# RobinWitch/SynTalker

Measured on AMD Instinct MI355X. Metric: denoising-steps/sec (128-frame clips), higher is better.
Workload: dtype bf16; 1 GPU; diffusion_rvqvae_128.yaml sampling: DDPM p_sample_loop steps (1000-step schedule), 1024 clips/GPU x (1536,1,32) latents, MDM denoiser 8x512, random-init; clips_per_gpu=1024, global_clips=1024, parallelism=clip-sharded x1, no collective, primed_steps=0, m_tile=auto

## Files before the change

### syntalker_amd/csrc/syn_kernels.hip

```cpp
#include <hip/hip_runtime.h>
#include <stdint.h>
#include <stdio.h>
#include <stdlib.h>
#include <string.h>

#include "syn_hip.h"

typedef __attribute__((ext_vector_type(8))) __bf16 bf16x8;
typedef __attribute__((ext_vector_type(4))) __bf16 bf16x4;
typedef __attribute__((ext_vector_type(4))) float f32x4;

#define MFMA16(a, b, c) __builtin_amdgcn_mfma_f32_16x16x32_bf16((a), (b), (c), 0, 0, 0)

namespace {

constexpr int kThreads = 512;
constexpr int kKT = 64;
constexpr int kNT = 512;

enum Epi { EPI_PLAIN = 0, EPI_IN = 1, EPI_QKV = 2, EPI_RESID = 3, EPI_GELU = 4, EPI_OUT = 5 };

struct GArgs {
    const __bf16* X; long x_chunk_stride; int ldx; int x_rows;
    const uint4* W; int K; int M;
// ... 1473 lines not shown
        if (hipGetDevice(&dev) != hipSuccess || dev < 0 || dev >= kMaxDevices) return true;
        if (done[dev]) return false;
        done[dev] = true;
        return true;
    }
};

void n128_setup() {
    static OncePerDevice once;
    if (once.first()) {
        allow_lds(k_gemm_n128, kN128Lds);
        allow_lds(k_gemm_pair<16, 2>, kN128Lds);
        allow_lds(k_gemm_and_pack<16, 2>, kN128Lds);
        allow_lds(k_gemm_quad_all, kN128Lds);
    }
}

struct StackInstance {
    int rows, tp;
    bool edit;
    void (*kernel)(SArgs);
    OncePerDevice once;
    int lds() const { return rows * 2048 + 4096; }
};
StackInstance* stack_instance(int rows, int tp, bool edit) {
    static StackInstance table[] = {
        {64, 0, false, k_stack<64>},          {32, 0, false, k_stack<32>},
        {64, 0, true,  k_stack<64, 0, true>}, {32, 0, true,  k_stack<32, 0, true>}, {32, 2, true, k_stack<32, 2, true>}, {32, 4, true, k_stack<32, 4, true>},
        {32, 2, false, k_stack<32, 2>},       {32, 4, false, k_stack<32, 4>},       {64, 2, false, k_stack<64, 2>},
    };
    for (StackInstance& i : table)
        if (i.rows == rows && i.tp == tp && i.edit == edit) return &i;
    return nullptr;
}

int launch_stack(const SArgs& a, int mt, hipStream_t s) {
    const bool edit = a.out.keep != nullptr;
    dim3 grid((a.M + mt - 1) / mt), block(kThreads);
    if (a.tp > 1) {
        if (!(mt == 32 || (mt == 64 && a.tp == 2)) || !a.sync || !a.xch) return fail_msg("stack: the tile-split mode needs 32-row tiles (or 64-row tiles split in two), ws_sync and ws_xch");
        grid.x = lat::kGroups * a.tp * ((a.tp_tiles + lat::kGroups - 1) / lat::kGroups);
        if (grid.x > 256) return fail_msg("stack: the tensor-parallel mode needs all its workgroups resident (<= 256)");
        if (edit && mt != 32) return fail_msg("stack: an edit takes split tiles of 32 rows only");
        if (a.tp != 2 && a.tp != 4) return fail_msg("stack: tile split over 2 or 4 workgroups only");
    }
    StackInstance* const k = stack_instance(mt, a.tp > 1 ? a.tp : 0, edit);
    if (!k) return fail_msg("stack: m_tile must be 32 or 64");
    if (k->once.first()) allow_lds(k->kernel, k->lds());
    hipLaunchKernelGGL(k->kernel, grid, block, k->lds(), s, a);
    return launched("k_stack launch");
}

}

#include "syn_stack_train.inc"
#include "syn_seq.inc"
#include "syn_cond.inc"
#include "syn_wavenc.inc"
#include "syn_train.inc"
#include "syn_conv_train.inc"
#include "syn_glue.inc"
#include "syn_rvq.inc"
#include "syn_rvq_train.inc"
#include "syn_pose.inc"
#include "syn_tmr.inc"
#include "syn_bert.inc"
#include "syn_skel.inc"
#include "syn_t2m.inc"
#include "syn_plms.inc"
#include "syn_bpd.inc"
#include "syn_guide.inc"
#include "syn_joints.inc"
#include "syn_mesh.inc"

namespace {

int launch_latency(const lat::LArgs& a, hipStream_t s) {
    static OncePerDevice once;
    if (once.first()) { allow_lds(lat::k_lat, lat::kLds); }
    hipLaunchKernelGGL(lat::k_lat, dim3(lat::kGroups * lat::kP), dim3(kThreads), lat::kLds, s, a);
    return launched("k_lat launch");
}

template <bool G, int NZ>
void launch_seq_as(const seq::QArgs& a, const dim3 grid, hipStream_t s) {
    static OncePerDevice once;
    if (once.first()) { allow_lds(seq::k_seq<G, NZ>, seq::kLds); }
    hipLaunchKernelGGL((seq::k_seq<G, NZ>), grid, dim3(seq::kThreads), seq::kLds, s, a);
}

int launch_seq(const seq::QArgs& a, hipStream_t s) {
    const dim3 grid(a.n_wg > 0 ? a.n_wg : seq_grid(a.R, a.V));
    const int nz = a.noise ? 1 : a.rng ? 2 : 0;
    if (a.V == 1) {
        if (nz == 2) launch_seq_as<false, 2>(a, grid, s); else if (nz == 1) launch_seq_as<false, 1>(a, grid, s); else launch_seq_as<false, 0>(a, grid, s);
    } else {
        if (nz == 2) launch_seq_as<true, 2>(a, grid, s); else if (nz == 1) launch_seq_as<true, 1>(a, grid, s); else launch_seq_as<true, 0>(a, grid, s);
    }
    return launched("k_seq launch");
}

}

extern "C" {

int syn_version(void) { return SYN_ABI_VERSION; }

void syn_debug_timing(long long* attn_buf, long long* mlp_buf) { g_dbg_attn = attn_buf; g_dbg_mlp = mlp_buf; }
const char* syn_last_error(void) { return g_err; }

int syn_pack_weight(const float* w, int32_t n, int32_t k, void* out_packed, void* stream) {
    if (!w || !out_packed || n % 16 || k % 32) return fail_msg("syn_pack_weight: need n%16==0, k%32==0, non-null pointers");
    const int total = (n / 16) * (k / 32) * 64;
    hipLaunchKernelGGL(k_pack, dim3((total + 255) / 256), dim3(256), 0, (hipStream_t)stream, w, n, k, (uint4*)out_packed);
    return launched("k_pack launch");
}

int syn_pack_weights(const syn_pack_job* jobs_dev, int32_t n_jobs, int64_t max_fragments, void* stream) {
    static_assert(sizeof(syn_pack_job) == sizeof(PackJob), "syn_pack_job is PackJob");
    if (!jobs_dev || n_jobs <= 0 || max_fragments <= 0) return fail_msg("syn_pack_weights: bad arguments");
    hipLaunchKernelGGL(k_pack_many, dim3((unsigned)((max_fragments * 64 + 255) / 256), n_jobs), dim3(256), 0, (hipStream_t)stream,
                       reinterpret_cast<const PackJob*>(jobs_dev));
    return launched("k_pack_many launch");
}

int syn_pack_weight_t(const void* s_kn, int32_t is_bf16, int32_t n, int32_t k, void* out_packed, void* stream) {
    if (!s_kn || !out_packed || n % 16 || k % 32) return fail_msg("syn_pack_weight_t: need n%16==0, k%32==0, non-null pointers");
    const int total = (n / 16) * (k / 32) * 64;
    if (is_bf16)
        hipLaunchKernelGGL(k_pack_t<__bf16>, dim3((total + 255) / 256), dim3(256), 0, (hipStream_t)stream, (const __bf16*)s_kn, n, k,
                           (uint4*)out_packed);
    else
        hipLaunchKernelGGL(k_pack_t<float>, dim3((total + 255) / 256), dim3(256), 0, (hipStream_t)stream, (const float*)s_kn, n, k,
                           (uint4*)out_packed);
    return launched("k_pack_t launch");
}

int syn_to_token_major(const float* x_bct, int32_t n_clips, float* out_f32, void* out_bf16, void* stream) {
    if (!x_bct || n_clips <= 0) return fail_msg("syn_to_token_major: bad arguments");
    hipLaunchKernelGGL(k_to_token_major, dim3(n_clips, SYN_C / 64), dim3(256), 0, (hipStream_t)stream, x_bct, out_f32,
                       (__bf16*)out_bf16);
    return launched("k_to_token_major launch");
}

int32_t syn_prefers_fragment_order(int32_t n_clips, int32_t n_variants) { return prefers_fragment_order(n_clips, n_variants, device_cus()); }

int syn_x_to_fragment(const float* x_bct, int32_t n_clips, float* out_f32, void* out_bf16, void* stream) {
    if (!x_bct || n_clips <= 0) return fail_msg("syn_x_to_fragment: bad arguments");
    hipLaunchKernelGGL(seq::k_x_to_fragment, dim3(n_clips, SYN_C / 32), dim3(256), 0, (hipStream_t)stream, x_bct, out_f32, (uint4*)out_bf16);
    return launched("k_x_to_fragment launch");
}

int syn_x_from_fragment(const float* x_frag, int32_t n_clips, float* out_bct, void* stream) {
    if (!x_frag || !out_bct || n_clips <= 0) return fail_msg("syn_x_from_fragment: bad arguments");
    hipLaunchKernelGGL(seq::k_x_from_fragment, dim3(n_clips, SYN_C / 32), dim3(256), 0, (hipStream_t)stream, x_frag, out_bct);
    return launched("k_x_from_fragment launch");
}

int syn_from_token_major(const float* x_btc, int32_t n_clips, float* out_bct, void* stream) {
    if (!x_btc || !out_bct || n_clips <= 0) return fail_msg("syn_from_token_major: bad arguments");
    hipLaunchKernelGGL(k_from_token_major, dim3(n_clips, SYN_C / 64), dim3(256), 0, (hipStream_t)stream, x_btc, out_bct);
    return launched("k_from_token_major launch");
}

int syn_axpby_rows(const float* x, const float* y, const float* coef_ab, const int32_t* t_row, int32_t n_clips,
                   int32_t per_clip, float* out, void* stream) {
    if (!x || !y || !coef_ab || !t_row || !out || n_clips <= 0 || per_clip % 4) return fail_msg("syn_axpby_rows: bad arguments");
    const long n4 = (long)n_clips * per_clip / 4;
    hipLaunchKernelGGL(k_axpby_rows, dim3((unsigned)((n4 + 255) / 256)), dim3(256), 0, (hipStream_t)stream, x, y, coef_ab,
                       t_row, n4, per_clip / 4, out);
    return launched("k_axpby_rows launch");
}

int syn_steps_advance(const int32_t* sched, int32_t* counter, int32_t* t_model, int32_t n_t_model, int32_t* t_coef, int32_t n_t_coef,
                      int32_t n_steps, void* stream) {
    if (!sched || !counter || !t_model || !t_coef || n_t_model <= 0 || n_t_coef <= 0 || n_steps <= 0)
        return fail_msg("syn_steps_advance: bad arguments");
    hipLaunchKernelGGL(k_step_advance, dim3(1), dim3(256), 0, (hipStream_t)stream, (const int*)sched, (int*)counter, (int*)t_model,
                       n_t_model, (int*)t_coef, n_t_coef, n_steps);
    return launched("k_step_advance launch");
// ... 452 lines not shown
```

### syntalker_amd/csrc/syn_seq.inc

```
namespace {
namespace seq {

typedef __attribute__((ext_vector_type(16))) float f32x16;
#define MFMA32(a, b, c) __builtin_amdgcn_mfma_f32_32x32x16_bf16((a), (b), (c), 0, 0, 0)

#ifndef SEQ_ABL
#define SEQ_ABL 0
#endif
#ifndef SEQ_ABL2
#define SEQ_ABL2 0
#endif
constexpr int kThreads = 256;
constexpr int kFragBytes = 1024;
#ifndef SEQ_CHUNK
#define SEQ_CHUNK 16
#endif
#ifndef SEQ_WIN
#define SEQ_WIN 4
#endif
#ifndef SEQ_SPREAD
#define SEQ_SPREAD 1
#endif
#ifndef SEQ_SCHED
#define SEQ_SCHED 0
#endif
constexpr int kChunkFrags = SEQ_CHUNK, kChunkBytes = kChunkFrags * kFragBytes;
constexpr int kPerWave = kChunkFrags / 4;
constexpr int kSlots = 80 / kChunkFrags, kLook = kSlots - 1;
constexpr int kRingBytes = kSlots * kChunkBytes;
constexpr int kBiasSet = 2048;
constexpr int kRingBase = 0;
constexpr int kBiasBase = kRingBytes;
constexpr int kSlabBase = kBiasBase + 2 * kBiasSet * 4;
constexpr int kSlabBytes = 4 * 4096;
constexpr int kLds = kSlabBase + 4 * kSlabBytes;
#if SEQ_CHUNK == 16
#define SEQ_WAIT_STEADY "s_waitcnt vmcnt(8)"
#define SEQ_WAIT_FIRST "s_waitcnt vmcnt(12)"
#else
#define SEQ_WAIT_STEADY "s_waitcnt vmcnt(14)"
#define SEQ_WAIT_FIRST "s_waitcnt vmcnt(16)"
#endif

struct QArgs {
    const char* tape; unsigned tape_chunks;
    const float* bias;
    const float* te; const float* rcos; const float* rsin;
    const float* cond; const int* t_model;
    const float* xt;
    const uint4* xb;
    const float* noise;
    const unsigned long long* rng; const float* coef; const int* t_coef;
    float* xn; uint4* xnb; float* x0;
    int R;
    int V;
    const float* cfg_w;
    int cfg_stride;
    int n_steps;
    int tm_stride, tc_stride;
    int wg0, n_wg;
    int dbg_step;
    unsigned skew;
    long long* dbg;
};

__device__ __forceinline__ void dma_frag(const char* src, unsigned lds_dst, unsigned lane16) {
    unsigned keep;
    asm volatile("s_mov_b32 %0, m0\n\t"
                 "s_mov_b32 m0, %2\n\t"
                 "s_nop 0\n\t"
                 "global_load_lds_dwordx4 %1, %3\n\t"
                 "s_mov_b32 m0, %0"
                 : "=&s"(keep) : "v"(lane16), "s"(lds_dst), "s"(src) : "memory");
}

template <int OFF>
__device__ __forceinline__ void dma_frag_at(const char* src, unsigned lds_dst, unsigned lane16) {
    asm volatile("s_mov_b32 m0, %1\n\t"
                 "s_nop 0\n\t"
                 "global_load_lds_dwordx4 %0, %2 offset:%c3"
                 :: "v"(lane16), "s"(lds_dst), "s"(src), "i"(OFF) : "memory");
}

#ifndef SEQ_DMA_POL
#define SEQ_DMA_POL 0
#endif
#if SEQ_DMA_POL == 1
#define SEQ_DMA_POLICY " nt"
#elif SEQ_DMA_POL == 2
#define SEQ_DMA_POLICY " sc1"
#elif SEQ_DMA_POL == 3
#define SEQ_DMA_POLICY " sc0"
#else
#define SEQ_DMA_POLICY ""
#endif
struct Ring {
    const char* tape;
    unsigned voff;
    unsigned dst;
    unsigned wq;
    unsigned voff0;
    unsigned lane16;
    unsigned cur, nxt;
    bf16x8 win[SEQ_WIN];
};
static_assert(SEQ_CHUNK == 16 && kPerWave == 4, "the pinned ring arithmetic below is written for 16-fragment chunks");

template <int OFF>
__device__ __forceinline__ void ring_dma(const Ring& r) {
    asm volatile("s_add_u32 m0, %1, %2\n\t"
                 "s_nop 0\n\t"
                 "global_load_lds_dwordx4 %0, %3 offset:%c4" SEQ_DMA_POLICY
                 :: "v"(r.voff), "s"(r.dst), "s"(r.wq), "s"(r.tape), "i"(OFF) : "memory", "scc");
}
__device__ __forceinline__ void ring_dma_i(const Ring& r, int i) {
    switch (i) {
        case 0: ring_dma<0>(r); break;
        case 1: ring_dma<1024>(r); break;
        case 2: ring_dma<2048>(r); break;
        default: ring_dma<3072>(r); break;
    }
}
__device__ __forceinline__ void ring_advance_dma(Ring& r) {
    const unsigned d = r.dst + kChunkBytes;
    r.dst = d == (unsigned)kRingBytes ? 0u : d;
    r.voff += kChunkBytes;
}
__device__ __forceinline__ void ring_next_base(Ring& r) {
    static_assert(kSlots == 5 && kRingBase == 0, "slot arithmetic");
    unsigned t = r.dst + 2 * kChunkBytes;
    t = t >= (unsigned)kRingBytes ? t - kRingBytes : t;
    r.nxt = r.lane16 + t;
}

__device__ __forceinline__ void bias_issue(const float* bias, const Ring& r, int set) {
    const char* src = reinterpret_cast<const char*>(bias + (size_t)set * kBiasSet) + r.wq / 2;
    const unsigned dst = kBiasBase + (set & 1) * (kBiasSet * 4) + r.wq / 2;
    dma_frag(src, dst, r.lane16);
    dma_frag(src + kFragBytes, dst + kFragBytes, r.lane16);
}

__device__ __forceinline__ void ring_boundary(Ring& r) {
    if (!(SEQ_ABL & 2)) {
        if (!(SEQ_ABL & 64)) asm volatile(SEQ_WAIT_STEADY ::: "memory");
        if (!(SEQ_ABL & 128)) __builtin_amdgcn_s_barrier();
    }
    r.cur = r.nxt;
}

__device__ __forceinline__ bf16x8 take(Ring& r, const char* lds, int& f) {
    if (f == 0) {
        const bf16x8 a = r.win[0];
        if (!(SEQ_ABL & 4)) r.win[0] = *reinterpret_cast<const bf16x8*>(lds + r.nxt + SEQ_WIN * kFragBytes);
        ring_boundary(r);
        __builtin_amdgcn_sched_barrier(0);
        f = 1;
        return a;
    }
    if (!(SEQ_ABL & 1) && (f & 3) == 2) ring_dma_i(r, f >> 2);
    if (f == 6) ring_next_base(r);
    if (f == 15) ring_advance_dma(r);
    const bf16x8 a = r.win[f & (SEQ_WIN - 1)];
    const int g = f + SEQ_WIN;
    if (!(SEQ_ABL & 4))
        r.win[f & (SEQ_WIN - 1)] = *reinterpret_cast<const bf16x8*>(lds + (g < kChunkFrags ? r.cur + g * kFragBytes : r.nxt + (g - kChunkFrags) * kFragBytes));
#if SEQ_SCHED == 0
    __builtin_amdgcn_sched_barrier(0);
#else
    __builtin_amdgcn_sched_group_barrier(0x100, 1, 0);
    __builtin_amdgcn_sched_group_barrier(0x008, 1, 0);
    __builtin_amdgcn_sched_group_barrier(0x002, SEQ_SCHED, 0);
#endif
    f = (f + 1) & (kChunkFrags - 1);
    return a;
}

__device__ __forceinline__ bf16x8 pack8(const f32x16& t, int c) {
    bf16x8 o;
#pragma unroll
    for (int e = 0; e < 8; ++e) o[e] = (__bf16)t[8 * c + e];
    return o;
}

__device__ __forceinline__ f32x16 zero16() {
    f32x16 z;
#pragma unroll
    for (int v = 0; v < 16; ++v) z[v] = 0.f;
    return z;
}

__device__ __forceinline__ f32x16 bias_tile(const char* lds, int set, int off, int tile, int hi) {
    unsigned at = (unsigned)(kBiasBase + (set & 1) * (kBiasSet * 4) + (off + 32 * tile + 4 * hi) * 4);
    asm volatile("" : "+v"(at));
    const float* b = reinterpret_cast<const float*>(lds + at);
    f32x16 o;
#pragma unroll
    for (int q = 0; q < 4; ++q) {
        const f32x4 v = *reinterpret_cast<const f32x4*>(b + 8 * q);
        o[4 * q] = v[0]; o[4 * q + 1] = v[1]; o[4 * q + 2] = v[2]; o[4 * q + 3] = v[3];
    }
    return o;
}

__device__ __forceinline__ f32x16 slab_load(const char* slab, int t) {
    f32x16 o;
#pragma unroll
    for (int q = 0; q < 4; ++q) {
        const f32x4 v = *reinterpret_cast<const f32x4*>(slab + (t * 4 + q) * 1024);
        o[4 * q] = v[0]; o[4 * q + 1] = v[1]; o[4 * q + 2] = v[2]; o[4 * q + 3] = v[3];
    }
    return o;
}
__device__ __forceinline__ void slab_store(char* slab, int t, const f32x16& v) {
#pragma unroll
    for (int q = 0; q < 4; ++q)
        *reinterpret_cast<f32x4*>(slab + (t * 4 + q) * 1024) = f32x4{v[4 * q], v[4 * q + 1], v[4 * q + 2], v[4 * q + 3]};
}

__device__ __forceinline__ float xor32(float v) { return __shfl_xor(v, 32); }

__device__ __forceinline__ float gelu_fast(float x) {
    if (SEQ_ABL2 & 1) return x;
    const float x2 = fminf(x * x, 64.0f);
    float t = fmaf(1.0142633e-3f, x2, -1.0677573e-1f);
    t = fmaf(t, x2, -2.3011213f);
    const float e = __builtin_amdgcn_exp2f(x * t);
    return nopk(x * __builtin_amdgcn_rcpf(1.0f + e));
}

struct NoFill { __device__ __forceinline__ void operator()(int) const {} };

__device__ __forceinline__ void slab_load_half(const char* slab, int t, int half, f32x16& o) {
#pragma unroll
    for (int q = 2 * half; q < 2 * half + 2; ++q) {
        const f32x4 v = *reinterpret_cast<const f32x4*>(slab + (t * 4 + q) * 1024);
        o[4 * q] = v[0]; o[4 * q + 1] = v[1]; o[4 * q + 2] = v[2]; o[4 * q + 3] = v[3];
    }
}
__device__ __forceinline__ void slab_store_quad(char* slab, int t, int q, const f32x16& v) {
    *reinterpret_cast<f32x4*>(slab + (t * 4 + q) * 1024) = f32x4{v[4 * q], v[4 * q + 1], v[4 * q + 2], v[4 * q + 3]};
}

template <int KC, int SPLIT = 0, typename Opnd, typename Fill = NoFill>
__device__ __forceinline__ void wide_of(Ring& r, const char* lds, f32x16 (&h)[12], char* slab, Opnd opnd, Fill fill = Fill()) {
    static_assert(SPLIT >= 0 && SPLIT < KC && (SPLIT == 0 || 12 * SPLIT >= 20), "slab loads must fit in front of their first use");
    constexpr int kLoad0 = SPLIT ? 12 * SPLIT - 12 : 0;
    constexpr int kStore0 = KC > 1 ? 16 * (KC - 1) + 4 : 16 * KC;
    f32x16 s[4];
    int f = 0, n = 0;
    auto mm = [&](f32x16& acc, int kc) {
        acc = MFMA32(take(r, lds, f), opnd(kc), acc);
        if (n >= kLoad0 && n < kLoad0 + 8) slab_load_half(slab, (n - kLoad0) >> 1, (n - kLoad0) & 1, s[(n - kLoad0) >> 1]);
        if (n >= kStore0 && n < kStore0 + 12) {
            const int j = n - kStore0, first = j < 4 ? 2 * j : 4 + j, cnt = j < 4 ? 2 : 1;
#pragma unroll
            for (int w = first; w < first + cnt; ++w) slab_store_quad(slab, w >> 2, w & 3, s[w >> 2]);
        }
        fill(n);
        ++n;
    };
    if constexpr (SPLIT > 0) {
#pragma unroll
        for (int kc = 0; kc < SPLIT; ++kc)
#pragma unroll
            for (int t = 0; t < 12; ++t) mm(h[t], kc);
#pragma unroll
        for (int kc = 0; kc < SPLIT; ++kc)
#pragma unroll
            for (int t = 0; t < 4; ++t) mm(s[t], kc);
    }
#pragma unroll
    for (int kc = SPLIT; kc < KC; ++kc) {
        if (KC > 1 && kc == KC - 1) {
#pragma unroll
            for (int t = 0; t < 4; ++t) mm(s[t], kc);
#pragma unroll
            for (int t = 0; t < 12; ++t) mm(h[t], kc);
        } else {
#pragma unroll
            for (int t = 0; t < 12; ++t) mm(h[t], kc);
#pragma unroll
            for (int t = 0; t < 4; ++t) mm(s[t], kc);
        }
    }
    if constexpr (KC == 1) {
#pragma unroll
        for (int t = 0; t < 4; ++t) slab_store(slab, t, s[t]);
    }
}

template <int KC, typename Fill = NoFill>
__device__ __forceinline__ void wide(Ring& r, const char* lds, f32x16 (&h)[12], char* slab, bf16x8 (&B)[KC], Fill fill = Fill()) {
    wide_of<KC, 0>(r, lds, h, slab, [&](int kc) { return B[kc]; }, fill);
}

template <bool SWAP, typename Fill = NoFill>
__device__ __forceinline__ void pair512(Ring& r, const char* lds, const bf16x8 (&B)[32], f32x16& a0, f32x16& a1, Fill fill = Fill()) {
    int f = 0;
#pragma unroll
    for (int kc = 0; kc < 32; ++kc) {
        const bf16x8 w0 = take(r, lds, f);
        a0 = SWAP ? MFMA32(B[kc], w0, a0) : MFMA32(w0, B[kc], a0);
        const bf16x8 w1 = take(r, lds, f);
        a1 = SWAP ? MFMA32(B[kc], w1, a1) : MFMA32(w1, B[kc], a1);
        fill(kc);
    }
}

typedef float f32x2 __attribute__((ext_vector_type(2)));
__device__ __forceinline__ f32x2 pk_add(f32x2 a, f32x2 b) { return a + b; }
__device__ __forceinline__ f32x2 pk_fma(f32x2 a, f32x2 b, f32x2 c) { return a * b + c; }

__device__ __forceinline__ void norm_to_operands(const f32x16 (&h)[12], const char* slab, bf16x8 (&xn)[32]) {
    if (SEQ_ABL2 & 16) {
#pragma unroll
        for (int i = 0; i < 32; ++i)
#pragma unroll
            for (int e = 0; e < 8; ++e) xn[i][e] = (__bf16)0.01f;
        return;
    }
    f32x2 s2 = {0.f, 0.f}, q2 = {0.f, 0.f};
#pragma unroll
    for (int t = 0; t < 16; ++t) {
        const f32x16 v = t < 12 ? h[t] : slab_load(slab, t - 12);
#pragma unroll
        for (int i = 0; i < 8; ++i) {
            const f32x2 p = {v[2 * i], v[2 * i + 1]};
            s2 = pk_add(s2, p);
            q2 = pk_fma(p, p, q2);
        }
    }
    float s = s2[0] + s2[1], q = q2[0] + q2[1];
    if (SEQ_ABL2 & 2) { s = 1.f; q = 600.f; }
    s += xor32(s); q += xor32(q);
    const float mean = s * (1.0f / 512.0f);
    const float var = fmaxf(q * (1.0f / 512.0f) - mean * mean, 0.f);
    const float rstd = rsqrtf(var + 1e-5f);
    const float nm = -mean * rstd;
    const f32x2 r2 = {rstd, rstd}, n2 = {nm, nm};
#pragma unroll
    for (int t = 0; t < 16; ++t) {
        const f32x16 v = t < 12 ? h[t] : slab_load(slab, t - 12);
#pragma unroll
        for (int c = 0; c < 2; ++c) {
            bf16x8 o;
#pragma unroll
            for (int e = 0; e < 4; ++e) {
                const f32x2 y = pk_fma(f32x2{v[8 * c + 2 * e], v[8 * c + 2 * e + 1]}, r2, n2);
                o[2 * e] = (__bf16)y[0]; o[2 * e + 1] = (__bf16)y[1];
            }
            xn[2 * t + c] = o;
        }
    }
}

using KArgs = const __attribute__((address_space(4))) QArgs;
#define KARGS(name) KArgs* name = reinterpret_cast<KArgs*>(reinterpret_cast<unsigned long long>(__builtin_amdgcn_kernarg_segment_ptr())); asm volatile("" : "+s"(name))

template <bool G, int NZ>
__global__ __launch_bounds__(kThreads) void k_seq(const QArgs) {
    extern __shared__ __attribute__((aligned(16))) char lds[];
    KARGS(a0);
    const int lane0 = threadIdx.x & 63;
    const int wave = __builtin_amdgcn_readfirstlane(threadIdx.x >> 6);
    int seq, cseq, var = 0, group0 = 0;
    bool live;
    if constexpr (!G) {
        seq = (a0->wg0 + (int)blockIdx.x) * 4 + wave;
        live = seq < a0->R;
        seq = live ? seq : a0->R - 1;
        cseq = seq;
    } else {
        const int V = a0->V, cpw = 4 / V;
        const int g = wave / V;
        seq = (a0->wg0 + (int)blockIdx.x) * cpw + g;
        live = g < cpw && seq < a0->R;
        var = live ? wave - g * V : -1;
        group0 = live ? g * V : 0;
        seq = live ? seq : a0->R - 1;
        cseq = (live ? var : 0) * a0->R + seq;
    }

    Ring r;
    r.tape = a0->tape; r.lane16 = (unsigned)lane0 * 16;
    r.wq = (unsigned)__builtin_amdgcn_readfirstlane(wave * (kPerWave * kFragBytes));
    r.voff0 = r.lane16 + r.wq;
    bias_issue(a0->bias, r, 0);
    r.voff = r.voff0; r.dst = kRingBase;
#pragma unroll 1
    for (int c = 0; c < kLook; ++c) {
#pragma unroll
        for (int i = 0; i < kPerWave; ++i) ring_dma_i(r, i);
        ring_advance_dma(r);
    }
    asm volatile(SEQ_WAIT_FIRST ::: "memory");
    __builtin_amdgcn_s_barrier();
    r.cur = r.lane16 + kRingBase;
    r.nxt = r.cur;
#pragma unroll
    for (int i = 0; i < SEQ_WIN; ++i) r.win[i] = *reinterpret_cast<const bf16x8*>(lds + kRingBase + r.lane16 + i * kFragBytes);
    if (a0->skew) {
        const unsigned n = (unsigned)(((unsigned long long)a0->skew * blockIdx.x) / gridDim.x);
        for (unsigned i = 0; i < n; ++i) __builtin_amdgcn_s_sleep(1);
        __builtin_amdgcn_s_barrier();
    }
    if (a0->dbg && wave == 0 && lane0 == 0) a0->dbg[(size_t)blockIdx.x * 32 + 0] = (long long)__builtin_readcyclecounter();

#pragma unroll 1
  for (int step = 0; step < a0->n_steps; ++step) {
    KARGS(a);
    if (step) {
        if constexpr (G) asm volatile("s_waitcnt vmcnt(0)" ::: "memory");
        __builtin_amdgcn_s_barrier();
        bias_issue(a->bias, r, 0);
        r.voff = r.voff0 + kLook * kChunkBytes;
        asm volatile("" : "+v"(r.voff));
    }
    int lane = lane0;
    asm volatile("" : "+v"(lane));
    const int hi = lane >> 5, tok = lane & 31;
    char* const slab = lds + kSlabBase + wave * kSlabBytes + lane * 16;
    const bool stamp = a->dbg && wave == 0 && lane == 0 && step == a->dbg_step;
    f32x16 h[12];
    {
        f32x16 g[16];
        const int ts = a->t_model[(size_t)step * a->tm_stride + cseq];
        const float* cp = a->cond + ((size_t)cseq * 32 + tok) * SYN_D + 4 * hi;
        const float* tp = a->te + (size_t)ts * SYN_D + 4 * hi;
#pragma unroll
        for (int t = 0; t < 16; ++t)
#pragma unroll
            for (int q = 0; q < 4; ++q) {
                const f32x4 c = *reinterpret_cast<const f32x4*>(cp + 32 * t + 8 * q);
                const f32x4 e = *reinterpret_cast<const f32x4*>(tp + 32 * t + 8 * q);
                g[t][4 * q] = c[0] + e[0]; g[t][4 * q + 1] = c[1] + e[1]; g[t][4 * q + 2] = c[2] + e[2]; g[t][4 * q + 3] = c[3] + e[3];
            }
        const uint4* xp = a->xb + (size_t)seq * (96 * 64) + lane;
        uint4 xq[8];
#pragma unroll
        for (int u = 0; u < 8; ++u) xq[u] = xp[u * 64];
#ifndef SEQ_IN_UNROLL
#define SEQ_IN_UNROLL 1
#endif
#pragma unroll SEQ_IN_UNROLL
        for (int j = 0; j < 12; ++j) {
#pragma unroll
            for (int u = 0; u < 8; ++u) {
                const bf16x8 b = __builtin_bit_cast(bf16x8, xq[u]);
                const int kn = min(j * 8 + u + 8, 95);
                if (!(SEQ_ABL & 32)) xq[u] = xp[(size_t)kn * 64];
                int f = 0;
#pragma unroll
                for (int t = 0; t < 16; ++t) g[t] = MFMA32(take(r, lds, f), b, g[t]);
            }
        }
        f32x4 cs[4], sn[4];
#pragma unroll
        for (int q = 0; q < 4; ++q) {
            cs[q] = *reinterpret_cast<const f32x4*>(a->rcos + tok * 32 + 8 * q + 4 * hi);
            sn[q] = *reinterpret_cast<const f32x4*>(a->rsin + tok * 32 + 8 * q + 4 * hi);
        }
#pragma unroll
        for (int p = 0; p < 8; ++p)
#pragma unroll
            for (int v = 0; v < 16; ++v) {
                const float u = g[2 * p][v], w = g[2 * p + 1][v], c = cs[v >> 2][v & 3], s = sn[v >> 2][v & 3];
                g[2 * p][v] = u * c - w * s;
                g[2 * p + 1][v] = w * c + u * s;
            }
#pragma unroll
        for (int t = 0; t < 12; ++t) h[t] = g[t];
#pragma unroll
        for (int t = 0; t < 4; ++t) slab_store(slab, t, g[12 + t]);
    }
    if (stamp) a->dbg[(size_t)blockIdx.x * 32 + 1] = (long long)__builtin_readcyclecounter();

    const float scale = 0.08838834764831845f * 1.4426950408889634f;
    auto make_ones = [&](bf16x8 (&o)[1]) {
        int hz = hi;
        asm volatile("" : "+v"(hz));
#pragma unroll
        for (int e = 0; e < 8; ++e) o[0][e] = (__bf16)((hz == 0 && e < 2) ? 1.0f : 0.0f);
    };
#pragma unroll 1
    for (int l = 0; l < SYN_LAYERS; ++l) {
        bf16x8 xn[32];
        norm_to_operands(h, slab, xn);
        {
            bf16x8 ones[1];
            make_ones(ones);
            wide<1>(r, lds, h, slab, ones);
        }
#pragma unroll 1
        for (int head = 0; head < SYN_HEADS; ++head) {
            bf16x8 qb[4][2];
#pragma unroll
            for (int p = 0; p < 2; ++p) {
                f32x16 a0 = bias_tile(lds, l, 128 * head, 2 * p, hi), a1 = bias_tile(lds, l, 128 * head, 2 * p + 1, hi);
                pair512<false>(r, lds, xn, a0, a1);
                qb[2 * p][0] = pack8(a0, 0); qb[2 * p][1] = pack8(a0, 1);
                qb[2 * p + 1][0] = pack8(a1, 0); qb[2 * p + 1][1] = pack8(a1, 1);
            }
            f32x16 s = zero16();
#pragma unroll
            for (int p = 0; p < 2; ++p) {
                f32x16 a0 = zero16(), a1 = zero16();
                pair512<false>(r, lds, xn, a0, a1);
                s = MFMA32(pack8(a0, 0), qb[2 * p][0], s);
                s = MFMA32(pack8(a0, 1), qb[2 * p][1], s);
                s = MFMA32(pack8(a1, 0), qb[2 * p + 1][0], s);
                s = MFMA32(pack8(a1, 1), qb[2 * p + 1][1], s);
            }
            float mx = s[0];
#pragma unroll
            for (int v = 1; v < 16; ++v) mx = fmaxf(mx, s[v]);
            mx = fmaxf(mx, xor32(mx));
            bf16x8 pb[2];
            float sum = 0.f;
#pragma unroll
            for (int v = 0; v < 16; ++v) {
                const __bf16 pv = (__bf16)__builtin_amdgcn_exp2f((s[v] - mx) * scale);
                pb[v >> 3][v & 7] = pv;
                sum += (float)pv;
            }
            sum += xor32(sum);
            const float inv = 1.0f / sum;
            bf16x8 ob[8];
#pragma unroll
            for (int p = 0; p < 2; ++p) {
                f32x16 a0 = zero16(), a1 = zero16();
                pair512<true>(r, lds, xn, a0, a1);
                f32x16 o0 = MFMA32(pack8(a0, 0), pb[0], zero16());
                o0 = MFMA32(pack8(a0, 1), pb[1], o0);
                f32x16 o1 = MFMA32(pack8(a1, 0), pb[0], zero16());
                o1 = MFMA32(pack8(a1, 1), pb[1], o1);
                o0 = o0 * inv; o1 = o1 * inv;
                ob[4 * p] = pack8(o0, 0); ob[4 * p + 1] = pack8(o0, 1);
                ob[4 * p + 2] = pack8(o1, 0); ob[4 * p + 3] = pack8(o1, 1);
            }
            wide<8>(r, lds, h, slab, ob);
        }
        bias_issue(a->bias, r, l + 1);
        norm_to_operands(h, slab, xn);
        {
            bf16x8 ones[1];
            make_ones(ones);
            wide<1>(r, lds, h, slab, ones);
        }
#pragma unroll 1
        for (int sl = 0; sl < SYN_FF / 128; ++sl) {
            bf16x8 hb[8];
            f32x16 a0 = bias_tile(lds, l, 512 + 128 * sl, 0, hi), a1 = bias_tile(lds, l, 512 + 128 * sl, 1, hi);
            pair512<false>(r, lds, xn, a0, a1);
            f32x16 b0 = bias_tile(lds, l, 512 + 128 * sl, 2, hi), b1 = bias_tile(lds, l, 512 + 128 * sl, 3, hi);
            pair512<false>(r, lds, xn, b0, b1, [&](int kc) {
                if (kc < 16) a0[kc] = gelu_fast(a0[kc]); else a1[kc - 16] = gelu_fast(a1[kc - 16]);
            });
            hb[0] = pack8(a0, 0); hb[1] = pack8(a0, 1); hb[2] = pack8(a1, 0); hb[3] = pack8(a1, 1);
            wide_of<8, 4>(r, lds, h, slab, [&](int kc) { return hb[kc]; }, [&](int i) {
                if (i < 16) b0[i] = gelu_fast(b0[i]);
                else if (i < 32) b1[i - 16] = gelu_fast(b1[i - 16]);
                else if (i == 32) hb[4] = pack8(b0, 0);
                else if (i == 33) hb[5] = pack8(b0, 1);
                else if (i == 34) hb[6] = pack8(b1, 0);
                else if (i == 35) hb[7] = pack8(b1, 1);
            });
        }
        if (stamp) a->dbg[(size_t)blockIdx.x * 32 + 2 + l] = (long long)__builtin_readcyclecounter();
    }

    {
        KARGS(a);
        bf16x8 hb[32];
#pragma unroll
        for (int t = 0; t < 16; ++t) {
            const f32x16 v = t < 12 ? h[t] : slab_load(slab, t - 12);
            hb[2 * t] = pack8(v, 0); hb[2 * t + 1] = pack8(v, 1);
        }
        const int tc = a->t_coef[(size_t)step * a->tc_stride + seq];
        const f32x4 cf = *reinterpret_cast<const f32x4*>(a->coef + (size_t)tc * 4);
        const size_t seq_f32 = (size_t)seq * (SYN_T * SYN_C * 4), seq_b16 = (size_t)seq * (SYN_T * SYN_C * 2);
        const char* const xt_s = reinterpret_cast<const char*>(a->xt) + seq_f32;
        char* const xn_s = reinterpret_cast<char*>(a->xn) + seq_f32;
        char* const xnb_s = reinterpret_cast<char*>(a->xnb) + seq_b16;
        char* const x0_s = a->x0 ? reinterpret_cast<char*>(a->x0) + seq_f32 : nullptr;
        [[maybe_unused]] const char* const nz_s = NZ == 1 ? reinterpret_cast<const char*>(a->noise) + seq_f32 : nullptr;
        [[maybe_unused]] unsigned long long seed = 0ull;
        [[maybe_unused]] unsigned long long idx4 = 0ull;
        if constexpr (NZ == 2) {
            seed = a->rng[0];
            idx4 = (a->rng[1] + (unsigned long long)seq) * (unsigned long long)(SYN_T * SYN_C / 4) + (unsigned long long)(tok * (SYN_C / 4) + hi);
        }
        int off_f = lane * 16, off_b = lane * 16;
        f32x16 acc_odd[2] = {zero16(), zero16()};
        f32x4 xt_odd[2][4], xo;
        [[maybe_unused]] const int nvar = G ? a->V : 1;
        [[maybe_unused]] unsigned gat = (unsigned)(kSlabBase + group0 * kSlabBytes + lane * 16);
        if constexpr (G) asm volatile("" : "+v"(gat));
        xo = f32x4{0.f, 0.f, 0.f, 0.f};
#pragma unroll
        for (int u = 0; u < 2; ++u)
#pragma unroll
            for (int q = 0; q < 4; ++q) xt_odd[u][q] = xo;
        auto fetch = [&](int off, f32x4 (&xt)[2][4]) {
#pragma unroll
            for (int u = 0; u < 2; ++u)
#pragma unroll
                for (int q = 0; q < 4; ++q)
                    xt[u][q] = (SEQ_ABL & 16) ? f32x4{1.f, 2.f, 3.f, 4.f} : *reinterpret_cast<const f32x4*>(xt_s + off + (u * 4 + q) * 1024);
        };
        auto quad = [&](int pr, int u, int q, const f32x16 (&pacc)[2], const f32x4 (&pxt)[2][4]) {
            const int at_f = off_f + (u * 4 + q) * 1024;
            f32x4 x0;
            if constexpr (!G) {
                x0 = f32x4{pacc[u][4 * q], pacc[u][4 * q + 1], pacc[u][4 * q + 2], pacc[u][4 * q + 3]};
            } else {
                const float* wc = a->cfg_w + (size_t)seq * a->cfg_stride + ((2 * pr + u) >> 4) * nvar;
                const unsigned at = gat + (unsigned)((pr & 1) * 8192 + (u * 4 + q) * 1024);
                x0 = *reinterpret_cast<const f32x4*>(lds + at) * wc[0];
#pragma unroll
                for (int v = 1; v < 4; ++v)
                    if (v < nvar) x0 = x0 + *reinterpret_cast<const f32x4*>(lds + at + v * kSlabBytes) * wc[v];
            }
            f32x4 xv;
            [[maybe_unused]] f32x4 z;
            if constexpr (NZ == 1) z = *reinterpret_cast<const f32x4*>(nz_s + at_f);
            if constexpr (NZ == 2) z = randn4<!G>(seed, (uint64_t)tc, idx4 + (unsigned long long)(8 * u + 2 * q));
#pragma unroll
            for (int e = 0; e < 4; ++e) {
                float v = fmaf(x0[e], cf[0], nopk(pxt[u][q][e] * cf[1]));
                if constexpr (NZ != 0) v = fmaf(z[e], cf[2], v);
                xv[e] = nopk(v);
            }
            if (live && (!(SEQ_ABL & 8) || a->R < 0)) {
                *reinterpret_cast<f32x4*>(xn_s + at_f) = xv;
                if (x0_s) *reinterpret_cast<f32x4*>(x0_s + at_f) = x0;
                if (q & 1) {
                    bf16x8 o;
#pragma unroll
                    for (int e = 0; e < 4; ++e) { o[e] = (__bf16)xo[e]; o[4 + e] = (__bf16)xv[e]; }
                    *reinterpret_cast<uint4*>(xnb_s + off_b + (u * 2 + (q >> 1)) * 1024) = __builtin_bit_cast(uint4, o);
                }
            }
            xo = xv;
        };
        auto advance = [&]() {
            off_f += 8192; off_b += 4096;
            if constexpr (NZ == 2) idx4 += 16;
        };
        if constexpr (!G) {
            auto pair = [&](int pr, bool first, f32x16 (&acc)[2], f32x4 (&cxt)[2][4], const f32x16 (&pacc)[2], const f32x4 (&pxt)[2][4]) {
                acc[0] = bias_tile(lds, SYN_LAYERS, 0, 2 * pr, hi); acc[1] = bias_tile(lds, SYN_LAYERS, 0, 2 * pr + 1, hi);
                fetch(first ? off_f : off_f + 8192, cxt);
                if (first) {
                    pair512<false>(r, lds, hb, acc[0], acc[1]);
                } else {
                    pair512<false>(r, lds, hb, acc[0], acc[1], [&](int kc) {
                        if ((kc & 3) == 0) quad(pr - 1, kc >> 4, (kc >> 2) & 3, pacc, pxt);
                    });
                    advance();
                }
            };
#pragma unroll 1
            for (int pp = 0; pp < 12; ++pp) {
                f32x16 acc_even[2];
                f32x4 xt_even[2][4];
                pair(2 * pp, pp == 0, acc_even, xt_even, acc_odd, xt_odd);
                pair(2 * pp + 1, false, acc_odd, xt_odd, acc_even, xt_even);
            }
        } else {
#pragma unroll 1
            for (int pr = 0; pr < 24; ++pr) {
                f32x16 acc0 = bias_tile(lds, SYN_LAYERS, 0, 2 * pr, hi), acc1 = bias_tile(lds, SYN_LAYERS, 0, 2 * pr + 1, hi);
                f32x4 cxt[2][4];
                fetch(pr == 0 ? off_f : off_f + 8192, cxt);
                if (pr == 0) {
                    pair512<false>(r, lds, hb, acc0, acc1);
                } else {
                    pair512<false>(r, lds, hb, acc0, acc1, [&](int kc) {
                        if ((kc & 3) == 0 && ((kc >> 3) % nvar) == var) quad(pr - 1, kc >> 4, (kc >> 2) & 3, acc_odd, xt_odd);
                    });
                    advance();
                }
                char* const mine = slab + (pr & 1) * 8192;
                slab_store(mine, 0, acc0);
                slab_store(mine, 1, acc1);
                asm volatile("s_waitcnt lgkmcnt(0)" ::: "memory");
#pragma unroll
                for (int u = 0; u < 2; ++u)
#pragma unroll
                    for (int q = 0; q < 4; ++q) xt_odd[u][q] = cxt[u][q];
            }
        }
        if constexpr (G) __builtin_amdgcn_s_barrier();
#pragma unroll
        for (int i = 0; i < 8; ++i)
            if (!G || ((i >> 1) % nvar) == var) quad(23, i >> 2, i & 3, acc_odd, xt_odd);
    }
    if (stamp) a->dbg[(size_t)blockIdx.x * 32 + 10] = (long long)__builtin_readcyclecounter();
  }
    if (a0->dbg && wave == 0 && lane0 == 0) a0->dbg[(size_t)blockIdx.x * 32 + 11] = (long long)__builtin_readcyclecounter();
    asm volatile("s_waitcnt vmcnt(0)" ::: "memory");
}

__global__ __launch_bounds__(256) void k_x_to_fragment(const float* __restrict__ x, float* __restrict__ of, uint4* __restrict__ ob) {
    __shared__ float tile[32][33];
    const int b = blockIdx.x, nf = blockIdx.y, tid = threadIdx.x;
#pragma unroll
    for (int i = 0; i < 4; ++i) {
        const int idx = tid + i * 256, c = idx >> 5, t = idx & 31;
        tile[c][t] = x[((size_t)b * SYN_C + 32 * nf + c) * 32 + t];
    }
    __syncthreads();
    {
        const int q = tid >> 6, lane = tid & 63, hi = lane >> 5, tk = lane & 31;
        f32x4 v;
#pragma unroll
        for (int r = 0; r < 4; ++r) v[r] = tile[8 * q + 4 * hi + r][tk];
        if (of) *reinterpret_cast<f32x4*>(of + (((size_t)b * 48 + nf) * 4 + q) * 256 + lane * 4) = v;
    }
    if (ob && tid < 128) {
        const int c = tid >> 6, lane = tid & 63, hi = lane >> 5, tk = lane & 31;
        bf16x8 o;
#pragma unroll
        for (int e = 0; e < 8; ++e) o[e] = (__bf16)tile[16 * c + 8 * (e >> 2) + 4 * hi + (e & 3)][tk];
        ob[((size_t)b * 48 + nf) * 128 + c * 64 + lane] = __builtin_bit_cast(uint4, o);
    }
}

__global__ __launch_bounds__(256) void k_x_from_fragment(const float* __restrict__ xf, float* __restrict__ out) {
    __shared__ float tile[32][33];
    const int b = blockIdx.x, nf = blockIdx.y, tid = threadIdx.x;
    {
        const int q = tid >> 6, lane = tid & 63, hi = lane >> 5, tk = lane & 31;
        const f32x4 v = *reinterpret_cast<const f32x4*>(xf + (((size_t)b * 48 + nf) * 4 + q) * 256 + lane * 4);
#pragma unroll
        for (int r = 0; r < 4; ++r) tile[8 * q + 4 * hi + r][tk] = v[r];
    }
    __syncthreads();
#pragma unroll
    for (int i = 0; i < 4; ++i) {
        const int idx = tid + i * 256, c = idx >> 5, t = idx & 31;
        out[((size_t)b * SYN_C + 32 * nf + c) * 32 + t] = tile[c][t];
    }
}

__global__ __launch_bounds__(kThreads) void k_mfma_rate(float* __restrict__ out, int iters) {
    extern __shared__ __attribute__((aligned(16))) char lds[];
    const int lane = threadIdx.x & 63;
    f32x16 acc[12];
#pragma unroll
    for (int i = 0; i < 12; ++i) acc[i] = zero16();
    bf16x8 a[4], b[4];
#pragma unroll
    for (int j = 0; j < 4; ++j)
#pragma unroll
        for (int e = 0; e < 8; ++e) {
            const unsigned ha = (unsigned)(lane * 8 + e + 977 * j) * 2654435761u, hb = (unsigned)(lane * 8 + e + 131 * j + 7) * 2246822519u;
            a[j][e] = (__bf16)(((float)(ha >> 16) - 32768.f) * (1.0f / 65536.f));
            b[j][e] = (__bf16)(((float)(hb >> 16) - 32768.f) * (1.0f / 65536.f));
        }
#pragma unroll 1
// ... 18 lines not shown
```

Baseline: 963,900 clip-steps/s.

## Pair LDS window reads, split DMA m0 setup, and use buffer stores in seq kernel

Parameterizes the weight-ring consumer per phase. Window refills are issued in pairs every other fragment, and the m0 setup of the LDS DMA is split from the global_load_lds issue so they can interleave with MFMA work. The final-projection operands are pinned to AGPRs, and the non-guided epilogue uses raw buffer stores whose range is set to zero when the tile should not store, replacing branches. A compile-time X0 template flag removes the x0 store when it is unused. This trades simpler scheduling for more template variants and register-pressure risk.

```diff
diff --git a/syntalker_amd/csrc/syn_kernels.hip b/syntalker_amd/csrc/syn_kernels.hip
--- a/syntalker_amd/csrc/syn_kernels.hip
+++ b/syntalker_amd/csrc/syn_kernels.hip
@@ -1579,20 +1579,25 @@
     return launched("k_lat launch");
 }
 
-template <bool G, int NZ>
+template <bool G, int NZ, bool X0>
 void launch_seq_as(const seq::QArgs& a, const dim3 grid, hipStream_t s) {
     static OncePerDevice once;
-    if (once.first()) { allow_lds(seq::k_seq<G, NZ>, seq::kLds); }
-    hipLaunchKernelGGL((seq::k_seq<G, NZ>), grid, dim3(seq::kThreads), seq::kLds, s, a);
+    if (once.first()) { allow_lds(seq::k_seq<G, NZ, X0>, seq::kLds); }
+    hipLaunchKernelGGL((seq::k_seq<G, NZ, X0>), grid, dim3(seq::kThreads), seq::kLds, s, a);
+}
+template <bool G, int NZ>
+void launch_seq_nz(const seq::QArgs& a, const dim3 grid, hipStream_t s) {
+    if constexpr (!G) { if (!a.x0) return launch_seq_as<G, NZ, false>(a, grid, s); }
+    launch_seq_as<G, NZ, true>(a, grid, s);
 }
 
 int launch_seq(const seq::QArgs& a, hipStream_t s) {
     const dim3 grid(a.n_wg > 0 ? a.n_wg : seq_grid(a.R, a.V));
     const int nz = a.noise ? 1 : a.rng ? 2 : 0;
     if (a.V == 1) {
-        if (nz == 2) launch_seq_as<false, 2>(a, grid, s); else if (nz == 1) launch_seq_as<false, 1>(a, grid, s); else launch_seq_as<false, 0>(a, grid, s);
+        if (nz == 2) launch_seq_nz<false, 2>(a, grid, s); else if (nz == 1) launch_seq_nz<false, 1>(a, grid, s); else launch_seq_nz<false, 0>(a, grid, s);
     } else {
-        if (nz == 2) launch_seq_as<true, 2>(a, grid, s); else if (nz == 1) launch_seq_as<true, 1>(a, grid, s); else launch_seq_as<true, 0>(a, grid, s);
+        if (nz == 2) launch_seq_nz<true, 2>(a, grid, s); else if (nz == 1) launch_seq_nz<true, 1>(a, grid, s); else launch_seq_nz<true, 0>(a, grid, s);
     }
     return launched("k_seq launch");
 }
diff --git a/syntalker_amd/csrc/syn_seq.inc b/syntalker_amd/csrc/syn_seq.inc
--- a/syntalker_amd/csrc/syn_seq.inc
+++ b/syntalker_amd/csrc/syn_seq.inc
@@ -17,6 +17,15 @@
 #endif
 #ifndef SEQ_WIN
 #define SEQ_WIN 4
+#endif
+#ifndef SEQ_PAIR
+#define SEQ_PAIR 2
+#endif
+#ifndef SEQ_M0FILL
+#define SEQ_M0FILL 5
+#endif
+#ifndef SEQ_HB_ACC
+#define SEQ_HB_ACC 1
 #endif
 #ifndef SEQ_SPREAD
 #define SEQ_SPREAD 1
@@ -104,6 +113,7 @@
     unsigned cur, nxt;
     bf16x8 win[SEQ_WIN];
 };
+template <bool PAIR, bool M0FILL> struct RingAs { Ring& r; static constexpr bool kPair = PAIR, kFill = M0FILL; };
 static_assert(SEQ_CHUNK == 16 && kPerWave == 4, "the pinned ring arithmetic below is written for 16-fragment chunks");
 
 template <int OFF>
@@ -121,6 +131,21 @@
         default: ring_dma<3072>(r); break;
     }
 }
+__device__ __forceinline__ void ring_dma_m0(const Ring& r) {
+    asm volatile("s_add_u32 m0, %0, %1" :: "s"(r.dst), "s"(r.wq) : "memory", "scc");
+}
+template <int OFF>
+__device__ __forceinline__ void ring_dma_go(const Ring& r) {
+    asm volatile("global_load_lds_dwordx4 %0, %1 offset:%c2" SEQ_DMA_POLICY :: "v"(r.voff), "s"(r.tape), "i"(OFF) : "memory");
+}
+__device__ __forceinline__ void ring_dma_go_i(const Ring& r, int i) {
+    switch (i) {
+        case 0: ring_dma_go<0>(r); break;
+        case 1: ring_dma_go<1024>(r); break;
+        case 2: ring_dma_go<2048>(r); break;
+        default: ring_dma_go<3072>(r); break;
+    }
+}
 __device__ __forceinline__ void ring_advance_dma(Ring& r) {
     const unsigned d = r.dst + kChunkBytes;
     r.dst = d == (unsigned)kRingBytes ? 0u : d;
@@ -148,22 +173,43 @@
     r.cur = r.nxt;
 }
 
-__device__ __forceinline__ bf16x8 take(Ring& r, const char* lds, int& f) {
+__device__ __forceinline__ bf16x8 win_read(const Ring& r, const char* lds, int g) {
+    return *reinterpret_cast<const bf16x8*>(lds + (g < kChunkFrags ? r.cur + g * kFragBytes : r.nxt + (g - kChunkFrags) * kFragBytes));
+}
+template <typename RingP>
+__device__ __forceinline__ bf16x8 take(RingP rp, const char* lds, int& f) {
+    constexpr bool PAIR = RingP::kPair, M0FILL = RingP::kFill;
+    Ring& r = rp.r;
+    static_assert(!PAIR || SEQ_WIN == 4, "paired reads are written for the four-deep window");
     if (f == 0) {
         const bf16x8 a = r.win[0];
-        if (!(SEQ_ABL & 4)) r.win[0] = *reinterpret_cast<const bf16x8*>(lds + r.nxt + SEQ_WIN * kFragBytes);
+        if (!(SEQ_ABL & 4)) {
+            if (PAIR) r.win[3] = *reinterpret_cast<const bf16x8*>(lds + r.nxt + 3 * kFragBytes);
+            r.win[0] = *reinterpret_cast<const bf16x8*>(lds + r.nxt + SEQ_WIN * kFragBytes);
+        }
         ring_boundary(r);
         __builtin_amdgcn_sched_barrier(0);
         f = 1;
         return a;
     }
-    if (!(SEQ_ABL & 1) && (f & 3) == 2) ring_dma_i(r, f >> 2);
-    if (f == 6) ring_next_base(r);
+    const bool dma = !(SEQ_ABL & 1) && (f & 3) == 2, split = dma && M0FILL && !(SEQ_ABL & 4);
+    if (dma) { if (split) ring_dma_m0(r); else ring_dma_i(r, f >> 2); }
+    if (f == (M0FILL ? 5 : 6)) ring_next_base(r);
     if (f == 15) ring_advance_dma(r);
-    const bf16x8 a = r.win[f & (SEQ_WIN - 1)];
-    const int g = f + SEQ_WIN;
-    if (!(SEQ_ABL & 4))
-        r.win[f & (SEQ_WIN - 1)] = *reinterpret_cast<const bf16x8*>(lds + (g < kChunkFrags ? r.cur + g * kFragBytes : r.nxt + (g - kChunkFrags) * kFragBytes));
+    bf16x8 a;
+    if (!PAIR) {
+        a = r.win[f & (SEQ_WIN - 1)];
+        if (!(SEQ_ABL & 4)) r.win[f & (SEQ_WIN - 1)] = win_read(r, lds, f + SEQ_WIN);
+        if (split) ring_dma_go_i(r, f >> 2);
+    } else if (f & 1) {
+        a = r.win[f & 3];
+        asm volatile("" :: "v"(a), "v"(r.win[(f + 1) & 3]));
+    } else {
+        a = r.win[f & 3];
+        if (!(SEQ_ABL & 4)) r.win[(f - 1) & 3] = win_read(r, lds, f + 3);
+        if (split) ring_dma_go_i(r, f >> 2);
+        if (!(SEQ_ABL & 4)) r.win[f & 3] = win_read(r, lds, f + 4);
+    }
 #if SEQ_SCHED == 0
     __builtin_amdgcn_sched_barrier(0);
 #else
@@ -173,6 +219,12 @@
 #endif
     f = (f + 1) & (kChunkFrags - 1);
     return a;
+}
+
+template <typename From, typename To>
+__device__ __forceinline__ void ring_hand_over(From, To to, const char* lds) {
+    if constexpr (From::kPair && !To::kPair)
+        if (!(SEQ_ABL & 4)) to.r.win[3] = *reinterpret_cast<const bf16x8*>(lds + to.r.nxt + 3 * kFragBytes);
 }
 
 __device__ __forceinline__ bf16x8 pack8(const f32x16& t, int c) {
@@ -241,8 +293,8 @@
     *reinterpret_cast<f32x4*>(slab + (t * 4 + q) * 1024) = f32x4{v[4 * q], v[4 * q + 1], v[4 * q + 2], v[4 * q + 3]};
 }
 
-template <int KC, int SPLIT = 0, typename Opnd, typename Fill = NoFill>
-__device__ __forceinline__ void wide_of(Ring& r, const char* lds, f32x16 (&h)[12], char* slab, Opnd opnd, Fill fill = Fill()) {
+template <int KC, int SPLIT = 0, typename Opnd, typename Fill = NoFill, typename RingP>
+__device__ __forceinline__ void wide_of(RingP r, const char* lds, f32x16 (&h)[12], char* slab, Opnd opnd, Fill fill = Fill()) {
     static_assert(SPLIT >= 0 && SPLIT < KC && (SPLIT == 0 || 12 * SPLIT >= 20), "slab loads must fit in front of their first use");
     constexpr int kLoad0 = SPLIT ? 12 * SPLIT - 12 : 0;
     constexpr int kStore0 = KC > 1 ? 16 * (KC - 1) + 4 : 16 * KC;
@@ -289,13 +341,13 @@
     }
 }
 
-template <int KC, typename Fill = NoFill>
-__device__ __forceinline__ void wide(Ring& r, const char* lds, f32x16 (&h)[12], char* slab, bf16x8 (&B)[KC], Fill fill = Fill()) {
+template <int KC, typename Fill = NoFill, typename RingP>
+__device__ __forceinline__ void wide(RingP r, const char* lds, f32x16 (&h)[12], char* slab, bf16x8 (&B)[KC], Fill fill = Fill()) {
     wide_of<KC, 0>(r, lds, h, slab, [&](int kc) { return B[kc]; }, fill);
 }
 
-template <bool SWAP, typename Fill = NoFill>
-__device__ __forceinline__ void pair512(Ring& r, const char* lds, const bf16x8 (&B)[32], f32x16& a0, f32x16& a1, Fill fill = Fill()) {
+template <bool SWAP, typename Fill = NoFill, typename RingP>
+__device__ __forceinline__ void pair512(RingP r, const char* lds, const bf16x8 (&B)[32], f32x16& a0, f32x16& a1, Fill fill = Fill()) {
     int f = 0;
 #pragma unroll
     for (int kc = 0; kc < 32; ++kc) {
@@ -357,7 +409,7 @@
 using KArgs = const __attribute__((address_space(4))) QArgs;
 #define KARGS(name) KArgs* name = reinterpret_cast<KArgs*>(reinterpret_cast<unsigned long long>(__builtin_amdgcn_kernarg_segment_ptr())); asm volatile("" : "+s"(name))
 
-template <bool G, int NZ>
+template <bool G, int NZ, bool X0>
 __global__ __launch_bounds__(kThreads) void k_seq(const QArgs) {
     extern __shared__ __attribute__((aligned(16))) char lds[];
     KARGS(a0);
@@ -382,6 +434,9 @@
     }
 
     Ring r;
+    const RingAs<!G && (SEQ_PAIR & 1), !G && (SEQ_M0FILL & 1)> r_in{r};
+    const RingAs<!G && (SEQ_PAIR & 2), !G && (SEQ_M0FILL & 2)> r_blk{r};
+    const RingAs<!G && (SEQ_PAIR & 4), !G && (SEQ_M0FILL & 4)> r_out{r};
     r.tape = a0->tape; r.lane16 = (unsigned)lane0 * 16;
     r.wq = (unsigned)__builtin_amdgcn_readfirstlane(wave * (kPerWave * kFragBytes));
     r.voff0 = r.lane16 + r.wq;
@@ -418,6 +473,7 @@
     }
     int lane = lane0;
     asm volatile("" : "+v"(lane));
+    if (step) ring_hand_over(r_out, r_in, lds);
     const int hi = lane >> 5, tok = lane & 31;
     char* const slab = lds + kSlabBase + wave * kSlabBytes + lane * 16;
     const bool stamp = a->dbg && wave == 0 && lane == 0 && step == a->dbg_step;
@@ -451,7 +507,7 @@
                 if (!(SEQ_ABL & 32)) xq[u] = xp[(size_t)kn * 64];
                 int f = 0;
 #pragma unroll
-                for (int t = 0; t < 16; ++t) g[t] = MFMA32(take(r, lds, f), b, g[t]);
+                for (int t = 0; t < 16; ++t) g[t] = MFMA32(take(r_in, lds, f), b, g[t]);
             }
         }
         f32x4 cs[4], sn[4];
@@ -482,6 +538,7 @@
 #pragma unroll
         for (int e = 0; e < 8; ++e) o[0][e] = (__bf16)((hz == 0 && e < 2) ? 1.0f : 0.0f);
     };
+    ring_hand_over(r_in, r_blk, lds);
 #pragma unroll 1
     for (int l = 0; l < SYN_LAYERS; ++l) {
         bf16x8 xn[32];
@@ -489,7 +546,7 @@
         {
             bf16x8 ones[1];
             make_ones(ones);
-            wide<1>(r, lds, h, slab, ones);
+            wide<1>(r_blk, lds, h, slab, ones);
         }
 #pragma unroll 1
         for (int head = 0; head < SYN_HEADS; ++head) {
@@ -497,7 +554,7 @@
 #pragma unroll
             for (int p = 0; p < 2; ++p) {
                 f32x16 a0 = bias_tile(lds, l, 128 * head, 2 * p, hi), a1 = bias_tile(lds, l, 128 * head, 2 * p + 1, hi);
-                pair512<false>(r, lds, xn, a0, a1);
+                pair512<false>(r_blk, lds, xn, a0, a1);
                 qb[2 * p][0] = pack8(a0, 0); qb[2 * p][1] = pack8(a0, 1);
                 qb[2 * p + 1][0] = pack8(a1, 0); qb[2 * p + 1][1] = pack8(a1, 1);
             }
@@ -505,7 +562,7 @@
 #pragma unroll
             for (int p = 0; p < 2; ++p) {
                 f32x16 a0 = zero16(), a1 = zero16();
-                pair512<false>(r, lds, xn, a0, a1);
+                pair512<false>(r_blk, lds, xn, a0, a1);
                 s = MFMA32(pack8(a0, 0), qb[2 * p][0], s);
                 s = MFMA32(pack8(a0, 1), qb[2 * p][1], s);
                 s = MFMA32(pack8(a1, 0), qb[2 * p + 1][0], s);
@@ -529,7 +586,7 @@
 #pragma unroll
             for (int p = 0; p < 2; ++p) {
                 f32x16 a0 = zero16(), a1 = zero16();
-                pair512<true>(r, lds, xn, a0, a1);
+                pair512<true>(r_blk, lds, xn, a0, a1);
                 f32x16 o0 = MFMA32(pack8(a0, 0), pb[0], zero16());
                 o0 = MFMA32(pack8(a0, 1), pb[1], o0);
                 f32x16 o1 = MFMA32(pack8(a1, 0), pb[0], zero16());
@@ -538,26 +595,26 @@
                 ob[4 * p] = pack8(o0, 0); ob[4 * p + 1] = pack8(o0, 1);
                 ob[4 * p + 2] = pack8(o1, 0); ob[4 * p + 3] = pack8(o1, 1);
             }
-            wide<8>(r, lds, h, slab, ob);
+            wide<8>(r_blk, lds, h, slab, ob);
         }
         bias_issue(a->bias, r, l + 1);
         norm_to_operands(h, slab, xn);
         {
             bf16x8 ones[1];
             make_ones(ones);
-            wide<1>(r, lds, h, slab, ones);
+            wide<1>(r_blk, lds, h, slab, ones);
         }
 #pragma unroll 1
         for (int sl = 0; sl < SYN_FF / 128; ++sl) {
             bf16x8 hb[8];
             f32x16 a0 = bias_tile(lds, l, 512 + 128 * sl, 0, hi), a1 = bias_tile(lds, l, 512 + 128 * sl, 1, hi);
-            pair512<false>(r, lds, xn, a0, a1);
+            pair512<false>(r_blk, lds, xn, a0, a1);
             f32x16 b0 = bias_tile(lds, l, 512 + 128 * sl, 2, hi), b1 = bias_tile(lds, l, 512 + 128 * sl, 3, hi);
-            pair512<false>(r, lds, xn, b0, b1, [&](int kc) {
+            pair512<false>(r_blk, lds, xn, b0, b1, [&](int kc) {
                 if (kc < 16) a0[kc] = gelu_fast(a0[kc]); else a1[kc - 16] = gelu_fast(a1[kc - 16]);
             });
             hb[0] = pack8(a0, 0); hb[1] = pack8(a0, 1); hb[2] = pack8(a1, 0); hb[3] = pack8(a1, 1);
-            wide_of<8, 4>(r, lds, h, slab, [&](int kc) { return hb[kc]; }, [&](int i) {
+            wide_of<8, 4>(r_blk, lds, h, slab, [&](int kc) { return hb[kc]; }, [&](int i) {
                 if (i < 16) b0[i] = gelu_fast(b0[i]);
                 else if (i < 32) b1[i - 16] = gelu_fast(b1[i - 16]);
                 else if (i == 32) hb[4] = pack8(b0, 0);
@@ -571,11 +628,15 @@
 
     {
         KARGS(a);
+        ring_hand_over(r_blk, r_out, lds);
         bf16x8 hb[32];
 #pragma unroll
         for (int t = 0; t < 16; ++t) {
             const f32x16 v = t < 12 ? h[t] : slab_load(slab, t - 12);
             hb[2 * t] = pack8(v, 0); hb[2 * t + 1] = pack8(v, 1);
+#if SEQ_HB_ACC
+            if constexpr (!G) asm volatile("" : "+a"(hb[2 * t]), "+a"(hb[2 * t + 1]));
+#endif
         }
         const int tc = a->t_coef[(size_t)step * a->tc_stride + seq];
         const f32x4 cf = *reinterpret_cast<const f32x4*>(a->coef + (size_t)tc * 4);
@@ -583,7 +644,14 @@
         const char* const xt_s = reinterpret_cast<const char*>(a->xt) + seq_f32;
         char* const xn_s = reinterpret_cast<char*>(a->xn) + seq_f32;
         char* const xnb_s = reinterpret_cast<char*>(a->xnb) + seq_b16;
-        char* const x0_s = a->x0 ? reinterpret_cast<char*>(a->x0) + seq_f32 : nullptr;
+        [[maybe_unused]] char* const x0_s = (G ? a->x0 != nullptr : X0) ? reinterpret_cast<char*>(a->x0) + seq_f32 : nullptr;
+        [[maybe_unused]] const bool stores = live && (!(SEQ_ABL & 8) || a->R < 0);
+        [[maybe_unused]] __amdgpu_buffer_rsrc_t xn_d, xnb_d, x0_d;
+        if constexpr (!G) {
+            xn_d = __builtin_amdgcn_make_buffer_rsrc(xn_s, 0, stores ? SYN_T * SYN_C * 4 : 0, 0x00020000);
+            xnb_d = __builtin_amdgcn_make_buffer_rsrc(xnb_s, 0, stores ? SYN_T * SYN_C * 2 : 0, 0x00020000);
+            if constexpr (X0) x0_d = __builtin_amdgcn_make_buffer_rsrc(x0_s, 0, stores ? SYN_T * SYN_C * 4 : 0, 0x00020000);
+        }
         [[maybe_unused]] const char* const nz_s = NZ == 1 ? reinterpret_cast<const char*>(a->noise) + seq_f32 : nullptr;
         [[maybe_unused]] unsigned long long seed = 0ull;
         [[maybe_unused]] unsigned long long idx4 = 0ull;
@@ -632,7 +700,17 @@
                 if constexpr (NZ != 0) v = fmaf(z[e], cf[2], v);
                 xv[e] = nopk(v);
             }
-            if (live && (!(SEQ_ABL & 8) || a->R < 0)) {
+            if constexpr (!G) {
+                typedef unsigned u32x4 __attribute__((ext_vector_type(4)));
+                __builtin_amdgcn_raw_buffer_store_b128(__builtin_bit_cast(u32x4, xv), xn_d, at_f, 0, 0);
+                if constexpr (X0) __builtin_amdgcn_raw_buffer_store_b128(__builtin_bit_cast(u32x4, x0), x0_d, at_f, 0, 0);
+                if (q & 1) {
+                    bf16x8 o;
+#pragma unroll
+                    for (int e = 0; e < 4; ++e) { o[e] = (__bf16)xo[e]; o[4 + e] = (__bf16)xv[e]; }
+                    __builtin_amdgcn_raw_buffer_store_b128(__builtin_bit_cast(u32x4, o), xnb_d, off_b + (u * 2 + (q >> 1)) * 1024, 0, 0);
+                }
+            } else if (live && (!(SEQ_ABL & 8) || a->R < 0)) {
                 *reinterpret_cast<f32x4*>(xn_s + at_f) = xv;
                 if (x0_s) *reinterpret_cast<f32x4*>(x0_s + at_f) = x0;
                 if (q & 1) {
@@ -653,9 +731,9 @@
                 acc[0] = bias_tile(lds, SYN_LAYERS, 0, 2 * pr, hi); acc[1] = bias_tile(lds, SYN_LAYERS, 0, 2 * pr + 1, hi);
                 fetch(first ? off_f : off_f + 8192, cxt);
                 if (first) {
-                    pair512<false>(r, lds, hb, acc[0], acc[1]);
+                    pair512<false>(r_out, lds, hb, acc[0], acc[1]);
                 } else {
-                    pair512<false>(r, lds, hb, acc[0], acc[1], [&](int kc) {
+                    pair512<false>(r_out, lds, hb, acc[0], acc[1], [&](int kc) {
                         if ((kc & 3) == 0) quad(pr - 1, kc >> 4, (kc >> 2) & 3, pacc, pxt);
                     });
                     advance();
@@ -675,9 +753,9 @@
                 f32x4 cxt[2][4];
                 fetch(pr == 0 ? off_f : off_f + 8192, cxt);
                 if (pr == 0) {
-                    pair512<false>(r, lds, hb, acc0, acc1);
+                    pair512<false>(r_out, lds, hb, acc0, acc1);
                 } else {
-                    pair512<false>(r, lds, hb, acc0, acc1, [&](int kc) {
+                    pair512<false>(r_out, lds, hb, acc0, acc1, [&](int kc) {
                         if ((kc & 3) == 0 && ((kc >> 3) % nvar) == var) quad(pr - 1, kc >> 4, (kc >> 2) & 3, acc_odd, xt_odd);
                     });
                     advance();
```

Measured after the change: 971,700 clip-steps/s, median of 6. No clear change (+0.8%).
